# RupertLuo/Valley

Measured on AMD Instinct MI355X. Metric: frames/sec ViT-L/14 encode + prefill tokens/sec (13B), higher is better.
Workload: dtype bf16

## Files before the change

valley_amd/csrc/gemm_skinny.hip:

```cpp
#include <cstdlib>
#include "common.hpp"
#include "../../include/valley_hip.h"

namespace {

constexpr int SK_UNROLL = 4;

template <int EPI, int NWV>
__global__ void __launch_bounds__(NWV * 64) gemm_skinny_kernel(const uint16_t* __restrict__ A, const uint16_t* __restrict__ W,
                                                               const float* __restrict__ bias, uint16_t* __restrict__ C, int M, int N,
                                                               int K, int lda, int ldw, int ldc) {
    __shared__ f32x4 red[NWV][4][64];
    const int tid = threadIdx.x, lane = tid & 63, wave = tid >> 6;
    const int l15 = lane & 15, g = lane >> 4;
    const int n0 = blockIdx.x * 32, m0 = blockIdx.y * 32;
    const int kq = K / NWV, kbeg = wave * kq;
    const uint16_t* a0 = A + (size_t)min(m0 + l15, M - 1) * lda + kbeg + g * 8;
    const uint16_t* a1 = A + (size_t)min(m0 + 16 + l15, M - 1) * lda + kbeg + g * 8;
    const uint16_t* w0 = W + (size_t)(n0 + l15) * ldw + kbeg + g * 8;
    const uint16_t* w1 = W + (size_t)(n0 + 16 + l15) * ldw + kbeg + g * 8;
    f32x4 acc[2][2];
#pragma unroll
    for (int i = 0; i < 2; ++i)
#pragma unroll
// ... 56 lines not shown
                acc[0][0] = mfma16(fw0[u], fa0[u], acc[0][0]);
                acc[0][1] = mfma16(fw1[u], fa0[u], acc[0][1]);
                acc[1][0] = mfma16(fw0[u], fa1[u], acc[1][0]);
                acc[1][1] = mfma16(fw1[u], fa1[u], acc[1][1]);
            }
        }
    }
#pragma unroll
    for (int i = 0; i < 2; ++i)
#pragma unroll
        for (int j = 0; j < 2; ++j) red[wave][2 * i + j][lane] = acc[i][j];
    __syncthreads();
    if (wave >= 4) return;
    f32x4 v = red[0][wave][lane];
#pragma unroll
    for (int w = 1; w < NWV; ++w) v += red[w][wave][lane];
    const int m = m0 + (wave >> 1) * 16 + l15, n = n0 + (wave & 1) * 16 + 4 * g;
    if (m >= M) return;
    if (bias) v += *(const f32x4*)(bias + n);
    if constexpr (EPI == VLY_EPI_QUICK_GELU) {
#pragma unroll
        for (int r = 0; r < 4; ++r) v[r] = x_sigmoid(v[r], 1.702f);
    }
    if constexpr (EPI == VLY_EPI_RELU) {
#pragma unroll
        for (int r = 0; r < 4; ++r) v[r] = fmaxf(v[r], 0.f);
    }
    u32x2 pk;
    pk[0] = pack_h2(v[0], v[1]);
    pk[1] = pack_h2(v[2], v[3]);
    *(u32x2*)(C + (size_t)m * ldc + n) = pk;
}

}

extern "C" int vly_gemm_skinny_bf16(const void* A, const void* W, const float* bias, void* C, int M, int N, int K, int lda, int ldw,
                                    int ldc, int epilogue, void* stream) {
    if (M <= 0 || M > 256 || N <= 0 || N % 32 || K < 128 || K % 128 || (K >= 2048 && K % 512) || lda % 8 || ldw % 8 || ldc % 4 || ((uintptr_t)A & 15) ||
        ((uintptr_t)W & 15) || ((uintptr_t)C & 7) || (bias && ((uintptr_t)bias & 15))) {
        vly_set_error("vly_gemm_skinny_bf16: unsupported shape/alignment M=%d N=%d K=%d lda=%d ldw=%d ldc=%d", M, N, K, lda, ldw, ldc);
        return -22;
    }
    static const bool narrow_only = getenv("VLY_SKINNY_WAVES") && atoi(getenv("VLY_SKINNY_WAVES")) == 4;
    const bool wide = K >= 2048 && !narrow_only;
    dim3 grid(N / 32, (M + 31) / 32), block(wide ? 1024 : 256);
    hipStream_t st = (hipStream_t)stream;
#define VLY_SKINNY(E)                                                                                                      \
    do {                                                                                                                   \
        if (wide)                                                                                                          \
            hipLaunchKernelGGL((gemm_skinny_kernel<E, 16>), grid, block, 0, st, (const uint16_t*)A, (const uint16_t*)W, bias,  \
                               (uint16_t*)C, M, N, K, lda, ldw, ldc);                                                      \
        else                                                                                                               \
            hipLaunchKernelGGL((gemm_skinny_kernel<E, 4>), grid, block, 0, st, (const uint16_t*)A, (const uint16_t*)W, bias,   \
                               (uint16_t*)C, M, N, K, lda, ldw, ldc);                                                      \
    } while (0)
    switch (epilogue) {
        case VLY_EPI_NONE: VLY_SKINNY(VLY_EPI_NONE); break;
        case VLY_EPI_QUICK_GELU: VLY_SKINNY(VLY_EPI_QUICK_GELU); break;
        case VLY_EPI_RELU: VLY_SKINNY(VLY_EPI_RELU); break;
        default: vly_set_error("vly_gemm_skinny_bf16: unsupported epilogue %d", epilogue); return -22;
    }
#undef VLY_SKINNY
    return vly_check_launch("vly_gemm_skinny_bf16");
}
```

valley_amd/agpr_audit.py:

```python
import re
import subprocess

AUDITED = {"gemm_bf16.hip": "gemm_p4_kernel", "gemm_p32.hip": "gemm_p32_kernel", "gemm_p16.hip": "gemm_p16_kernel"}


def audit_asm(asm_path, kern):
    asm = open(asm_path).read().splitlines()
    bad = kernels = 0
    report = []
    i = 0
    areg = re.compile(r"\ba(\[(\d+|0x[0-9a-f]+)(:(\d+|0x[0-9a-f]+))?\]|\d+\b)")
    while i < len(asm):
        m = re.match(r"^(_ZN\S*" + kern + r"\S*):", asm[i])
        if not m:
            i += 1
            continue
        name = subprocess.run(["c++filt", m.group(1)], capture_output=True, text=True).stdout.strip()
        name = re.sub(r"\(anonymous namespace\)::", "", name).split("(")[0].replace("void ", "")
        j = i + 1
        in_asm = False
        outside, n_mfma, n_rd, n_mfma_compiler = [], 0, 0, 0
        while j < len(asm) and "s_endpgm" not in asm[j]:
            ln = asm[j]
            if ";;#ASMSTART" in ln:
                in_asm = True
            elif ";;#ASMEND" in ln:
                in_asm = False
            else:
                code = ln.split(";")[0]
                if in_asm:
                    if "v_mfma" in code:
                        n_mfma += 1
                    if "v_accvgpr_read" in code:
                        n_rd += 1
                elif areg.search(code) and not code.strip().startswith("."):
                    outside.append((j - i, code.strip()))
                    if "v_mfma" in code:
                        n_mfma_compiler += 1
                if "scratch_" in code:
                    outside.append((j - i, code.strip()))
            j += 1
        named = [int(x, 0) for ln in asm[i:j] for x in re.findall(r"\ba\[(?:\d+|0x[0-9a-f]+):(\d+|0x[0-9a-f]+)\]", ln.split(";")[0])]
        desc = "\n".join(asm[j:j + 120])
        nf = re.search(r"\.amdhsa_next_free_vgpr\s+(\d+)", desc)
        ao = re.search(r"\.amdhsa_accum_offset\s+(\d+)", desc)
        lit = n_mfma > 0 and n_mfma_compiler == 0 and "v_mfma" not in "\n".join(c for _, c in outside)
        if lit and named and nf and ao and int(nf.group(1)) - int(ao.group(1)) < max(named) + 1:
            outside.append((0, f"descriptor allocates {int(nf.group(1)) - int(ao.group(1))} accumulation registers, the asm names a{max(named)}"))
        if lit and not (nf and ao):
            outside.append((0, "kernel descriptor not found behind the kernel"))
        if n_mfma_compiler:
            lit = False
        if lit:
            kernels += 1
            status = "ok" if not outside else "FAIL"
            report.append(f"{name:48s} mfma {n_mfma:4d}  acc reads {n_rd:4d}  compiler AGPR / scratch instructions: {len(outside)}  {status}")
            for off, code in outside[:8]:
                report.append(f"    +{off}: {code}")
            bad += len(outside)
        i = j
    return report, kernels, bad
```

valley_amd/csrc/gemm_bf16.hip:

```cpp
#include <cmath>
#include <cstdlib>
#include <cstring>
#include <type_traits>
#include "common.hpp"
#include "../../include/valley_hip.h"

int vly_tile_order_m_fast(int M, int N, int K, int tiles_m, int tiles_n) {
    const double a = (double)M * K, w = (double)N * K;
    const double n_fast = a + w * (tiles_m < 8 ? tiles_m : 8);
    const double m_fast = w + a * (tiles_n < 8 ? tiles_n : 8);
    return m_fast < n_fast;
}

int vly_tile_group_height(int M, int N, int K, int tiles_m, int tiles_n, int BM, int BN, int wg_per_cu) {
    static const int forced = getenv("VLY_TILE_GM") ? atoi(getenv("VLY_TILE_GM")) : 0;
    static const int forced_max_m = getenv("VLY_TILE_GM_MAXM") ? atoi(getenv("VLY_TILE_GM_MAXM")) : 0x7fffffff;
    if (forced > 0 && M <= forced_max_m) return forced < tiles_m ? forced : tiles_m;
    static const bool grouped = !(getenv("VLY_TILE_GROUPED") && atoi(getenv("VLY_TILE_GROUPED")) == 0);
    if (!grouped) return vly_tile_order_m_fast(M, N, K, tiles_m, tiles_n) ? tiles_m : 1;
    if (tiles_n <= 8 && 8 % tiles_n == 0 && !vly_tile_order_m_fast(M, N, K, tiles_m, tiles_n)) return 1;
    const double conc = 32.0 * wg_per_cu;
    int gm = (int)(sqrt(conc * BN / BM) + 0.5);
    if (gm < 1) gm = 1;
    if (gm >= tiles_m || tiles_m <= gm + gm / 2) return tiles_m;
// ... 39 lines not shown
constexpr int P8_RD2_START = 1;
constexpr int P8_RD2_STRIDE = 2;
constexpr int P4_M0_LEAD = 2;
#ifndef VLY_P4_ROLL
#define VLY_P4_ROLL 1
#endif
#ifndef VLY_P4_ROLL_MASK
#define VLY_P4_ROLL_MASK 0x09
#endif
#ifndef VLY_P4_LIT
#define VLY_P4_LIT 1
#endif
#ifndef VLY_P4_CHAIN
#define VLY_P4_CHAIN 0
#endif
#ifndef VLY_P4_LATE
#define VLY_P4_LATE 0
#endif
#ifndef VLY_P4_DROPSTORE
#define VLY_P4_DROPSTORE 0
#endif
#ifndef VLY_P4_TIMING
#define VLY_P4_TIMING 0
#endif
#ifndef VLY_EXPERIMENTAL
#define VLY_EXPERIMENTAL 0
#endif

#if VLY_FP16
#define VLY_MFMA16_NAME "v_mfma_f32_16x16x32_f16"
#else
#define VLY_MFMA16_NAME "v_mfma_f32_16x16x32_bf16"
#endif
VLY_DEVICE void mfma16_lit(int blk, const bf16x8& a, const bf16x8& b) {
    asm volatile(VLY_MFMA16_NAME " a[%2:%3], %0, %1, a[%2:%3]" ::"v"(a), "v"(b), "i"(4 * blk), "i"(4 * blk + 3));
}
VLY_DEVICE void mfma16_lit_zero(int blk, const bf16x8& a, const bf16x8& b) {
    asm volatile(VLY_MFMA16_NAME " a[%2:%3], %0, %1, 0" ::"v"(a), "v"(b), "i"(4 * blk), "i"(4 * blk + 3));
}
VLY_DEVICE f32x4 acc_read_lit(int blk) {
    f32x4 v;
    asm volatile("v_accvgpr_read_b32 %0, a[%4]\n\tv_accvgpr_read_b32 %1, a[%5]\n\tv_accvgpr_read_b32 %2, a[%6]\n\tv_accvgpr_read_b32 %3, a[%7]"
                 : "=v"(v[0]), "=v"(v[1]), "=v"(v[2]), "=v"(v[3])
                 : "i"(4 * blk), "i"(4 * blk + 1), "i"(4 * blk + 2), "i"(4 * blk + 3));
    return v;
}
#define VLY_A8(n) "a" #n "0", "a" #n "1", "a" #n "2", "a" #n "3", "a" #n "4", "a" #n "5", "a" #n "6", "a" #n "7", "a" #n "8", "a" #n "9"
#define VLY_ALL_AGPRS                                                                                                                  \
    "a0", "a1", "a2", "a3", "a4", "a5", "a6", "a7", "a8", "a9", VLY_A8(1), VLY_A8(2), VLY_A8(3), VLY_A8(4), VLY_A8(5), VLY_A8(6), VLY_A8(7), \
        VLY_A8(8), VLY_A8(9), VLY_A8(10), VLY_A8(11), VLY_A8(12), VLY_A8(13), VLY_A8(14), VLY_A8(15), VLY_A8(16), VLY_A8(17), VLY_A8(18),   \
        VLY_A8(19), VLY_A8(20), VLY_A8(21), VLY_A8(22), VLY_A8(23), VLY_A8(24), "a250", "a251", "a252", "a253", "a254", "a255"

template <int MI, int NI, int N1, int S1, int D1, int N2, int S2, int D2, int N3, int S3, int D3, int N4, int S4, int D4, int MODE = 0,
          typename F1, typename F2, typename F3, typename F4, typename ACC>
VLY_DEVICE void phase_4w4(ACC& acc, const bf16x8 (&af)[MI], const bf16x8 (&wf)[NI], F1&& f1, F2&& f2, F3&& f3, F4&& f4) {
    __builtin_amdgcn_sched_barrier(0);
#pragma unroll
    for (int k = 0; k < N4; ++k)
        if (S4 + k * D4 < 0) f4(k);
#pragma unroll
    for (int i = 0; i < MI; ++i) {
#pragma unroll
        for (int j = 0; j < NI; ++j) {
            if constexpr (MODE == 3) mfma16_lit_zero(i * NI + j, wf[j], af[i]);
            else if constexpr (MODE == 2) mfma16_lit(i * NI + j, wf[j], af[i]);
            else acc[i][j] = mfma16(wf[j], af[i], acc[i][j]);
            const int t = i * NI + j;
            if (N1 > 0 && t >= S1 && (t - S1) % D1 == 0 && (t - S1) / D1 < N1) {
                __builtin_amdgcn_sched_barrier(0);
                f1((t - S1) / D1);
                __builtin_amdgcn_sched_barrier(0);
            }
            if (N3 > 0 && t >= S3 && (t - S3) % D3 == 0 && (t - S3) / D3 < N3) {
                __builtin_amdgcn_sched_barrier(0);
                f3((t - S3) / D3);
                __builtin_amdgcn_sched_barrier(0);
            }
            if (N4 > 0 && t >= S4 && (t - S4) % D4 == 0 && (t - S4) / D4 < N4) {
                __builtin_amdgcn_sched_barrier(0);
                f4((t - S4) / D4);
                __builtin_amdgcn_sched_barrier(0);
            }
            if (N2 > 0 && t >= S2 && (t - S2) % D2 == 0 && (t - S2) / D2 < N2) {
                __builtin_amdgcn_sched_barrier(0);
// ... 644 lines not shown
#undef VLY_FRAG_ROW
#undef VLY_FRAG_COL
#undef EPI_NH

VLY_DEVICE f32x4 acc_read(const f32x4& a) {
    f32x4 v;
    asm volatile("v_accvgpr_read_b32 %0, %4\n\tv_accvgpr_read_b32 %1, %5\n\tv_accvgpr_read_b32 %2, %6\n\tv_accvgpr_read_b32 %3, %7"
                 : "=v"(v[0]), "=v"(v[1]), "=v"(v[2]), "=v"(v[3])
                 : "a"(a[0]), "a"(a[1]), "a"(a[2]), "a"(a[3]));
    return v;
}
VLY_DEVICE void acc_read_pairs(const f32x4& a, f32x2& even, f32x2& odd) {
    asm volatile("v_accvgpr_read_b32 %0, %4\n\tv_accvgpr_read_b32 %1, %5\n\tv_accvgpr_read_b32 %2, %6\n\tv_accvgpr_read_b32 %3, %7"
                 : "=v"(even[0]), "=v"(odd[0]), "=v"(even[1]), "=v"(odd[1])
                 : "a"(a[0]), "a"(a[1]), "a"(a[2]), "a"(a[3]));
}

struct P4Cursor {
    int tile, k, kend, u, r;
};
constexpr int P4_SK_MAX_WAYS = 8;
constexpr unsigned P4_SK_SPIN_LIMIT = 1u << 24;
constexpr int P4_SK_ERR_FLAG = 4000;

template <int BM, int BN, int EPI, int OUT, bool SK>
__global__ void __launch_bounds__(256)
gemm_p4_kernel(const uint16_t* __restrict__ A, const uint16_t* __restrict__ W, const float* __restrict__ bias,
               const float* __restrict__ R, void* __restrict__ Cv, int M, int N, int K, int lda, int ldw, int ldc, int ldr,
               int tiles_m, int tiles_n, int gm, RopeArgs rp, float* __restrict__ slabs, unsigned* __restrict__ flags,
               unsigned epoch, int sk_S) {
    constexpr int WM = BM / 2, WN = BN / 2, NT = 256;
    constexpr bool SKT = SK && BM != 256;
    constexpr int MI = WM / 16, NI = WN / 16;
    constexpr int A_BYTES = BM * 128, W_BYTES = BN * 128, STAGE = A_BYTES + W_BYTES;
    constexpr int PA = BM * 8 / NT, PW = BN * 8 / NT, NS = PA + PW;
    static_assert(BM * 8 % NT == 0 && BN * 8 % NT == 0 && NI % 4 == 0, "tile/threads mismatch");
    constexpr int T = MI * NI, BAR_AT = MI + NI + P8_BAR_GAP, GL1_START = BAR_AT + 2;
    constexpr int GL_STRIDE = (2 * T - GL1_START) / NS;
    constexpr int N1 = (T - GL1_START + GL_STRIDE - 1) / GL_STRIDE, N2 = NS - N1;
    constexpr int GL2_START = GL1_START + N1 * GL_STRIDE - T;
    static_assert(GL1_START < T && GL_STRIDE >= 1 && N2 >= 0 && GL2_START + (N2 - 1) * GL_STRIDE < T, "piece schedule");
    __shared__ __attribute__((aligned(16))) char smem[2 * STAGE];
#if VLY_P4_TIMING
    __shared__ unsigned long long tstamp[64];
    int tsn = 0;
#define VLY_STAMP()                                                                            \
    do {                                                                                       \
        if (!SK && threadIdx.x == 0 && tsn < 64) tstamp[tsn] = __builtin_readcyclecounter();  \
        ++tsn;                                                                                 \
    } while (0)
#else
#define VLY_STAMP() do {} while (0)
#endif

    const int tid = threadIdx.x, lane = tid & 63;
    const int wave = __builtin_amdgcn_readfirstlane(tid >> 6);
    const int l15 = lane & 15, g = lane >> 4;
    const int ntiles = tiles_m * tiles_n, G = (int)gridDim.x;
    const int nk = K / BK;
    __builtin_assume(nk >= 2);
    const uint32_t wk = ldw < 0 ? (uint32_t)((N + 63) >> 6) * 4096u : (uint32_t)BK;
    auto tile_origin = [&](int t, int& m0, int& n0) {
        const int xcd = t & 7, qd = ntiles >> 3, rm = ntiles & 7;
        const int swz = (xcd < rm ? xcd * (qd + 1) : rm * (qd + 1) + (xcd - rm) * qd) + (t >> 3);
        const int gsz = gm * tiles_n, grp = swz / gsz, first = grp * gm;
        const int gh = min(gm, tiles_m - first), rr = swz - grp * gsz;
// ... 115 lines not shown
#pragma unroll
        for (int j = 0; j < NI; ++j) {
            w0[j] = *(const bf16x8*)(st + rdW + j * 2048 + sw0);
            w1[j] = *(const bf16x8*)(st + rdW + j * 2048 + sw1);
        }
#pragma unroll
        for (int i = 0; i < CH; ++i) {
            a0[i] = *(const bf16x8*)(st + rdA + i * 2048 + sw0);
            a1[i] = *(const bf16x8*)(st + rdA + i * 2048 + sw1);
        }
    };

#pragma unroll
    for (int q = 0; q < NS; ++q) piece(0, q);
    advance_load();
#pragma unroll
    for (int q = 0; q < NS; ++q) piece(1, q);
    advance_load();
    asm volatile("s_waitcnt vmcnt(%0)" ::"i"(NS) : "memory");
    __builtin_amdgcn_s_barrier();
    if constexpr (CHAIN) chain_preload(smem);
    else {
        auto r0 = rd_step0(smem);
#pragma unroll
        for (int k = 0; k < MI + NI; ++k) r0(k);
    }
    [[maybe_unused]] const __amdgpu_buffer_rsrc_t rsC =
        __builtin_amdgcn_make_buffer_rsrc(Cv, 0, (uint32_t)M * (uint32_t)ldc * (OUT == VLY_OUT_BF16 ? 2u : 4u), 0x00020000);
    int buf = 0;
    constexpr bool LIT = VLY_P4_LIT != 0 && !SK && OUT == VLY_OUT_BF16 && EPI != VLY_EPI_QKV_ROPE;
    constexpr bool ROLL = VLY_P4_ROLL != 0 && LIT && !CHAIN && ((VLY_P4_ROLL_MASK >> EPI) & 1) != 0;
    constexpr int NST_ = EPI == VLY_EPI_SWIGLU ? NI / 4 : NI / 2;
    static_assert(!ROLL || N1 + MI * NST_ <= 63, "vmcnt is a 6-bit count");
    if constexpr (LIT) asm volatile("" ::: VLY_ALL_AGPRS);
    f32x4 acc[MI][NI];
    bool wave_live = false;
    auto ktile = [&](auto first_c, bool relaxed = false) {
        constexpr bool FIRST = decltype(first_c)::value;
        const char* cur = smem + buf * STAGE;
        const char* nxt = smem + (buf ^ 1) * STAGE;
        __builtin_amdgcn_s_waitcnt(0xc07f);
        if constexpr (CHAIN) {
            if (wave_live) {
                phase_seq<CT1, CR1, 0, 1, CN1, CGL1, CGLS, 1, CBAR, 1, CN1, CGL1 - P4_M0_LEAD, CGLS>(
                    [&](int t) {
                        const int i = t / (2 * NI), j = (t % (2 * NI)) >> 1, st = t & 1;
                        if (FIRST && st == 0) mfma16_lit_zero(i * NI + j, w0[j], a0[i]);
                        else if (st == 0) mfma16_lit(i * NI + j, w0[j], a0[i]);
                        else mfma16_lit(i * NI + j, w1[j], a1[i]);
                    },
                    [&](int k) {
                        const int i = CH + (k >> 1);
                        if (k & 1) a1[i < MI ? i : 0] = *(const bf16x8*)(cur + rdA + i * 2048 + sw1);
                        else a0[i < MI ? i : 0] = *(const bf16x8*)(cur + rdA + i * 2048 + sw0);
                    },
                    [&](int q) { piece_ld(q); }, bar_a, [&](int q) { piece_m0(buf, q); });
            } else {
                __builtin_amdgcn_s_barrier();
#pragma unroll
                for (int q = 0; q < CN1; ++q) piece(buf, q);
            }
            asm volatile("s_waitcnt vmcnt(%0)" ::"i"(CN1) : "memory");
            __builtin_amdgcn_s_barrier();
            if (wave_live) {
                constexpr int CW = 2 * (MI - CH);
                phase_seq<CT2, 2 * CH, 1, 2, CN2, CGL2, CGLS, NI, CW - 1, CW, CN2, CGL2 - P4_M0_LEAD, CGLS>(
                    [&](int t) {
// ... 86 lines not shown
        if constexpr (OUT == VLY_OUT_BF16 && EPI != VLY_EPI_QKV_ROPE) {
            {
                const uint32_t rowb = (uint32_t)(em0 + wm0 + l15) * (uint32_t)ldc * 2u;
#pragma unroll
                for (int s = 0; s < NST; ++s) {
                    const int n = EPI == VLY_EPI_SWIGLU ? ((en0 + wn0) >> 1) + (4 * s + g) * 8
                                                        : en0 + wn0 + (2 * s + (g & 1)) * 16 + (g & 2) * 4;
                    vo[s] = rowb + (n + 8 <= No && !VLY_P4_DROPSTORE ? (uint32_t)n * 2u : 0x80000000u);
                }
            }
            if constexpr (EPI != VLY_EPI_SWIGLU) {
#pragma unroll
                for (int j = 0; j < NI; ++j) {
                    const int n = en0 + wn0 + j * 16 + g * 4;
                    bv[j] = f32x4{0.f, 0.f, 0.f, 0.f};
                    if (bias) bv[j] = *(const f32x4*)(bias + min(n, N - 4));
                }
            }
        }
    };
    [[maybe_unused]] auto epi_row = [&](int i, auto&& hook, auto defer_c) {
        constexpr bool DEFER = decltype(defer_c)::value;
        if constexpr (OUT == VLY_OUT_BF16 && EPI != VLY_EPI_QKV_ROPE) {
            if constexpr (EPI == VLY_EPI_SWIGLU) {
#pragma unroll
                for (int jq = 0; jq < NI / 4; ++jq) {
                    f32x2 gt[4], up[4], e[4];
#pragma unroll
                    for (int jj = 0; jj < 4; ++jj) {
                        if constexpr (SKT) {
                            const f32x4 v = acc_read(acc[i][4 * jq + jj]) + slab_term(i, 4 * jq + jj);
                            gt[jj] = f32x2{v[0], v[2]};
                            up[jj] = f32x2{v[1], v[3]};
                        } else if constexpr (LIT) {
                            const f32x4 v = acc_read_lit(i * NI + 4 * jq + jj);
                            gt[jj] = f32x2{v[0], v[2]};
                            up[jj] = f32x2{v[1], v[3]};
                        } else acc_read_pairs(acc[i][4 * jq + jj], gt[jj], up[jj]);
                    }
                    if constexpr (SKT) sk_next(i + 1, 4 * jq, 4);
                    hook(8 * jq + 0);
#pragma unroll
                    for (int q = 0; q < 4; ++q) e[q] = gt[q] * -1.4426950408889634f;
                    hook(8 * jq + 1);
#pragma unroll
                    for (int q = 0; q < 2; ++q) e[q] = f32x2{__builtin_amdgcn_exp2f(e[q][0]), __builtin_amdgcn_exp2f(e[q][1])};
                    hook(8 * jq + 2);
#pragma unroll
                    for (int q = 2; q < 4; ++q) e[q] = f32x2{__builtin_amdgcn_exp2f(e[q][0]), __builtin_amdgcn_exp2f(e[q][1])};
                    hook(8 * jq + 3);
#pragma unroll
                    for (int q = 0; q < 4; ++q) e[q] += 1.f;
#pragma unroll
                    for (int q = 0; q < 2; ++q) e[q] = f32x2{__builtin_amdgcn_rcpf(e[q][0]), __builtin_amdgcn_rcpf(e[q][1])};
                    hook(8 * jq + 4);
#pragma unroll
                    for (int q = 2; q < 4; ++q) e[q] = f32x2{__builtin_amdgcn_rcpf(e[q][0]), __builtin_amdgcn_rcpf(e[q][1])};
                    hook(8 * jq + 5);
#pragma unroll
                    for (int q = 0; q < 4; ++q) gt[q] *= e[q];
#pragma unroll
                    for (int q = 0; q < 4; ++q) gt[q] *= up[q];
                    hook(8 * jq + 6);
                    uint32_t d[4];
#pragma unroll
                    for (int jj = 0; jj < 4; ++jj) d[jj] = pack_h2(gt[jj][0], gt[jj][1]);
// ... 370 lines not shown
                    }
                }
            }
        }
        }
        if constexpr (SK) {
            if (!cur_next_seg(cc)) break;
            ct = cc.tile;
        } else {
            if (ct + G >= ntiles) break;
            ct += G;
        }
        tile_origin(ct, cm0, cn0);
        if constexpr (CHAIN) chain_preload(smem + buf * STAGE);
        else {
            auto r0 = rd_step0(smem + buf * STAGE);
#pragma unroll
            for (int k = 0; k < MI + NI; ++k) r0(k);
        }
    }
    VLY_STAMP();
    asm volatile("s_waitcnt vmcnt(0)" ::: "memory");
#if VLY_P4_TIMING
    VLY_STAMP();
    if (!SK && threadIdx.x == 0 && blockIdx.x < 64 && slabs) {
        unsigned long long* o = (unsigned long long*)slabs + (size_t)blockIdx.x * 65;
        o[0] = (unsigned long long)tsn;
        for (int q = 0; q < 64 && q < tsn; ++q) o[1 + q] = tstamp[q];
    }
#endif
}
#undef VLY_STAMP

#if VLY_P4_TIMING
static void* vlydbg_p4_buffer() {
    static void* buf = [] { void* p = nullptr; (void)hipMalloc(&p, 64 * 65 * 8); (void)hipMemset(p, 0, 64 * 65 * 8); return p; }();
    return buf;
}
extern "C" int vlydbg_p4_timing_read(unsigned long long* host) {
    return (int)hipMemcpy(host, vlydbg_p4_buffer(), 64 * 65 * 8, hipMemcpyDeviceToHost);
}
#endif
struct P4SkArgs {
    float* slabs;
    unsigned* flags;
    unsigned epoch;
    int slab_cap;
};

template <int BM, int BN, bool SK = false>
int launch_p4(const void* A, const void* W, const float* bias, const float* R, void* C, int M, int N, int K, int lda, int ldw,
              int ldc, int ldr, int epi, int out, hipStream_t st, const RopeArgs* rope = nullptr, const P4SkArgs* sk = nullptr) {
    const int tm = (M + BM - 1) / BM, tn = (N + BN - 1) / BN;
    const int gm = vly_tile_group_height(M, N, K, tm, tn, BM, BN, 1);
    const int No = epi == VLY_EPI_SWIGLU ? N >> 1 : N;
    const int vec_ok = (out == VLY_OUT_BF16 && ldc % 8 == 0 && ((uintptr_t)C & 15) == 0 && !R && No % 8 == 0 &&
                        (size_t)M * (size_t)ldc * 2 < ((size_t)1 << 31)) ? 1 : 0;
    if (out == VLY_OUT_BF16 && !vec_ok) return 1;
    static const int cus = [] {
        int dev = 0, n = 0;
        (void)hipGetDevice(&dev);
        (void)hipDeviceGetAttribute(&n, hipDeviceAttributeMultiprocessorCount, dev);
        if (getenv("VLY_P4_GRID")) n = atoi(getenv("VLY_P4_GRID"));
        return n > 0 ? n / 8 * 8 : 256;
    }();
    const int tiles = tm * tn;
    int sk_S = 1;
    if constexpr (SK) {
        const int rem = tiles % cus, rem8 = (rem + 7) & ~7, nk = K / BK;
        float best = 1e30f;
        for (int S = 1; S <= P4_SK_MAX_WAYS && rem > 0; ++S) {
            if (S > 1 && ((S - 1) * rem8 > sk->slab_cap || nk / S < 2 || (S - 1) * ((nk + S - 1) / S) >= nk)) continue;
            const float cost = (float)((S * rem8 + cus - 1) / cus) / (float)S + 0.06f * (float)(S - 1);
            if (cost < best - 1e-6f) { best = cost; sk_S = S; }
        }
        static const int pin = [] { const char* e = getenv("VLY_P4_SK_S"); return e ? atoi(e) : 0; }();
        if (pin > 0 && rem > 0 && (pin == 1 || ((pin - 1) * rem8 <= sk->slab_cap && nk / pin >= 2))) sk_S = pin;
    }
    dim3 grid(SK || tiles >= cus ? cus : tiles), block(256);
#if VLY_P4_TIMING
    P4SkArgs dbg{(float*)vlydbg_p4_buffer(), nullptr, 0u, 0};
    if (!sk) sk = &dbg;
#endif
#define VLY_P4_LAUNCH(E, O)                                                                                                  \
    hipLaunchKernelGGL((gemm_p4_kernel<BM, BN, E, O, SK>), grid, block, 0, st, (const uint16_t*)A, (const uint16_t*)W, bias, R, C, M, \
                       N, K, lda, ldw, ldc, ldr, tm, tn, gm, rope ? *rope : RopeArgs{}, sk ? sk->slabs : nullptr,                 \
                       sk ? sk->flags : nullptr, sk ? sk->epoch : 0u, sk_S)
    if (epi == VLY_EPI_NONE && out == VLY_OUT_BF16) VLY_P4_LAUNCH(VLY_EPI_NONE, VLY_OUT_BF16);
    else if (epi == VLY_EPI_NONE && out == VLY_OUT_F32) VLY_P4_LAUNCH(VLY_EPI_NONE, VLY_OUT_F32);
    else if (epi == VLY_EPI_QUICK_GELU && out == VLY_OUT_BF16) VLY_P4_LAUNCH(VLY_EPI_QUICK_GELU, VLY_OUT_BF16);
    else if (epi == VLY_EPI_SWIGLU && out == VLY_OUT_BF16) VLY_P4_LAUNCH(VLY_EPI_SWIGLU, VLY_OUT_BF16);
    else if (epi == VLY_EPI_RELU && out == VLY_OUT_BF16) VLY_P4_LAUNCH(VLY_EPI_RELU, VLY_OUT_BF16);
    else if (!SK && epi == VLY_EPI_QKV_ROPE && out == VLY_OUT_BF16 && rope) {
        if constexpr (!SK) VLY_P4_LAUNCH(VLY_EPI_QKV_ROPE, VLY_OUT_BF16);
    } else {
        vly_set_error("vly_gemm_bf16: unsupported epilogue/out_dtype combination (%d,%d) for the persistent tiles", epi, out);
        return -22;
    }
#undef VLY_P4_LAUNCH
    return vly_check_launch("vly_gemm_bf16");
}

template <int BM, int BN, int WM, int WN, int PIPE>
int launch_tile(const void* A, const void* W, const float* bias, const float* R, void* C, int M, int N, int K,
                int lda, int ldw, int ldc, int ldr, int epi, int out, hipStream_t st, void* C2 = nullptr,
                const RopeArgs* rope = nullptr) {
    constexpr int NT = (BM / WM) * (BN / WN) * 64;
    const int tm = (M + BM - 1) / BM, tn = (N + BN - 1) / BN;
    constexpr int STAGE_B = (BM + BN) * 128 * ((PIPE == 6 || PIPE == 7) ? 3 : 2);
    const int gm = vly_tile_group_height(M, N, K, tm, tn, BM, BN, STAGE_B <= 80 * 1024 ? 2 : 1);
    static const bool frag_only = getenv("VLY_EPILOGUE") && !strcmp(getenv("VLY_EPILOGUE"), "frag");
    static const bool lds_only = getenv("VLY_EPILOGUE") && !strcmp(getenv("VLY_EPILOGUE"), "lds");
    int wide = (out == VLY_OUT_BF16 && ldc % 8 == 0 && ((uintptr_t)C & 15) == 0 && !frag_only) ? 1 : 0;
    if (wide && PIPE == 8 && epi != VLY_EPI_QKV_ROPE && !lds_only) wide = 2;
    const int ksplit = C2 ? 2 : 1;
    dim3 grid(tm * tn * ksplit), block(NT);
#define VLY_GEMM_LAUNCH(E, O)                                                                         \
    hipLaunchKernelGGL((gemm_kernel<BM, BN, WM, WN, E, O, PIPE>), grid, block, 0, st, (const uint16_t*)A,   \
                       (const uint16_t*)W, bias, R, C, M, N, K, lda, ldw, ldc, ldr, tm, tn, gm, wide, ksplit, C2, rope ? *rope : RopeArgs{})
    if (epi == VLY_EPI_NONE && out == VLY_OUT_BF16) VLY_GEMM_LAUNCH(VLY_EPI_NONE, VLY_OUT_BF16);
    else if (epi == VLY_EPI_NONE && out == VLY_OUT_F32) VLY_GEMM_LAUNCH(VLY_EPI_NONE, VLY_OUT_F32);
    else if (epi == VLY_EPI_QUICK_GELU && out == VLY_OUT_BF16) VLY_GEMM_LAUNCH(VLY_EPI_QUICK_GELU, VLY_OUT_BF16);
    else if (epi == VLY_EPI_SWIGLU && out == VLY_OUT_BF16) VLY_GEMM_LAUNCH(VLY_EPI_SWIGLU, VLY_OUT_BF16);
    else if (epi == VLY_EPI_RELU && out == VLY_OUT_BF16) VLY_GEMM_LAUNCH(VLY_EPI_RELU, VLY_OUT_BF16);
    else if (epi == VLY_EPI_QKV_ROPE && out == VLY_OUT_BF16 && rope) {
        if constexpr (BN % 128 == 0) {
            if (!wide) { vly_set_error("vly_gemm_bf16_qkv_rope: qkv rows must be 16-byte aligned"); return -22; }
            VLY_GEMM_LAUNCH(VLY_EPI_QKV_ROPE, VLY_OUT_BF16);
        } else {
            vly_set_error("vly_gemm_bf16_qkv_rope: this tile is not a multiple of 128 columns wide");
            return -22;
        }
    }
// ... 97 lines not shown
        case 5: return launch_tile<192, 256, 96, 64, 0>(VLY_TILE_ARGS);
        case 73: return launch_tile<256, 128, 64, 64, 6>(VLY_TILE_ARGS);
        case 74: return launch_tile<128, 256, 64, 64, 6>(VLY_TILE_ARGS);
        case 76: return launch_tile<192, 192, 96, 48, 6>(VLY_TILE_ARGS);
        case 6: return launch_tile<192, 192, 96, 48, 0>(VLY_TILE_ARGS);
        case 83: return launch_tile<256, 128, 64, 64, 7>(VLY_TILE_ARGS);
        case 84: return launch_tile<128, 256, 64, 64, 7>(VLY_TILE_ARGS);
        case 86: return launch_tile<192, 192, 96, 48, 7>(VLY_TILE_ARGS);
        case 7: return launch_tile<128, 192, 64, 48, 0>(VLY_TILE_ARGS);
        case 8: return launch_tile<192, 128, 96, 32, 0>(VLY_TILE_ARGS);
        case 9: return launch_tile<256, 256, 64, 64, 0>(VLY_TILE_ARGS);
        case 93: return launch_tile<256, 128, 64, 32, 6>(VLY_TILE_ARGS);
        case 94: return launch_tile<128, 256, 32, 64, 6>(VLY_TILE_ARGS);
        case 497: {
            const int rc = rope || C2 ? 1 : valley_p16_gemm(A, W, bias, residual, C, M, N, K, lda, ldw, ldc, epilogue, out_dtype, st);
            return rc == 1 ? run_tile(197, tile_hint, VLY_TILE_ARGS_RAW) : rc;
        }
        case 397:
        case 398: {
            const int rc = rope || C2 ? 1 : valley_p32_gemm(A, W, bias, residual, C, M, N, K, lda, ldw, ldc, epilogue, out_dtype, st, t == 398);
            return rc == 1 ? run_tile(197, tile_hint, VLY_TILE_ARGS_RAW) : rc;
        }
        case 197:
        case 198:
        case 199:
            if (C2) { vly_set_error("vly_gemm_bf16: tile_hint %d does not take the split-K pair", tile_hint); return -22; }
            if (K < 2 * BK) return run_tile(t - 100, tile_hint, VLY_TILE_ARGS_RAW);
            {
                const int rc = t == 197 ? launch_p4<256, 256>(A, W, bias, residual, C, M, N, K, lda, ldw, ldc, ldr, epilogue, out_dtype, st, rope)
                               : t == 198 ? launch_p4<224, 256>(A, W, bias, residual, C, M, N, K, lda, ldw, ldc, ldr, epilogue, out_dtype, st, rope)
                                          : launch_p4<192, 256>(A, W, bias, residual, C, M, N, K, lda, ldw, ldc, ldr, epilogue, out_dtype, st, rope);
                return rc == 1 ? run_tile(t - 100, tile_hint, VLY_TILE_ARGS_RAW) : rc;
            }
        case 97:
        case 98:
        case 99:
            if (t == 97) return launch_tile<256, 256, 128, 128, 8>(VLY_TILE_ARGS);
            if (t == 98) return launch_tile<224, 256, 112, 128, 8>(VLY_TILE_ARGS);
            return launch_tile<192, 256, 96, 128, 8>(VLY_TILE_ARGS);
        case 51: return launch_tile<256, 256, 128, 64, 4>(VLY_TILE_ARGS);
        case 53: return launch_tile<256, 128, 64, 64, 4>(VLY_TILE_ARGS);
        case 54: return launch_tile<128, 256, 64, 64, 4>(VLY_TILE_ARGS);
        case 55: return launch_tile<192, 256, 96, 64, 4>(VLY_TILE_ARGS);
        default: vly_set_error("vly_gemm_bf16: bad tile_hint %d", tile_hint); return -22;
    }
#endif
#undef VLY_TILE_ARGS
#undef VLY_TILE_ARGS_RAW
}

extern "C" int vly_gemm_bf16(const void* A, const void* W, const float* bias, const float* residual, void* C,
                             int M, int N, int K, int lda, int ldw, int ldc, int ldr, int epilogue,
                             int out_dtype, int tile_hint, void* stream) {
    if (M <= 0 || N <= 0 || K <= 0) { vly_set_error("vly_gemm_bf16: empty problem"); return -22; }
    const bool wpacked = ldw == VLY_LDW_PACKED64;
    if (K % BK || lda % 8 || (ldw % 8 || (ldw <= 0 && !wpacked)) || N % 4 || ldc % 2 || (epilogue == VLY_EPI_SWIGLU && N % 8) ||
        ((uintptr_t)A & 15) || ((uintptr_t)W & 15) || ((uintptr_t)C & 7) ||
        (residual && (ldr % 4 || ((uintptr_t)residual & 15))) || (bias && ((uintptr_t)bias & 15))) {
        vly_set_error("vly_gemm_bf16: unsupported shape/alignment M=%d N=%d K=%d lda=%d ldw=%d ldc=%d ldr=%d",
                      M, N, K, lda, ldw, ldc, ldr);
        return -22;
    }
    if ((size_t)M * lda >= (1ull << 31) || (wpacked ? (size_t)((N + 63) / 64 * 64) * K : (size_t)N * ldw) >= (1ull << 31)) {
        vly_set_error("vly_gemm_bf16: operand exceeds 2^31 elements (32-bit byte offsets)");
        return -22;
    }
// ... 47 lines not shown
```

valley_amd/ops.py:

```python
from __future__ import annotations

import os
import threading
from typing import Optional

import torch

from . import lib as _lib
from . import runtime

EPI_NONE, EPI_QUICK_GELU, EPI_SWIGLU, EPI_RELU, EPI_QKV_ROPE = 0, 1, 2, 3, 4
OUT_BF16, OUT_F32 = 0, 1
POOL_MEAN, POOL_MAX, POOL_IMPORTANCE = 0, 1, 2


_RECORDER = None
TILE_NAMES = {1: "256, 256, 128, 64", 2: "128, 128, 64, 64", 3: "256, 128, 64, 64", 4: "128, 256, 64, 64",
              5: "192, 256, 96, 64", 6: "192, 192, 96, 48", 7: "128, 192, 64, 48",
              8: "192, 128, 96, 32", 9: "256, 256, 64, 64"}
TILE_SPECIAL = {93: ("256, 128, 64, 32", 6), 94: ("128, 256, 32, 64", 6),
                97: ("256, 256, 128, 128", 8), 98: ("224, 256, 112, 128", 8),
                99: ("192, 256, 96, 128", 8),
                197: ("p4 256, 256", 8), 198: ("p4 224, 256", 8), 199: ("p4 192, 256", 8)}

# ... 47 lines not shown

def _gemm_common(fn_name, a, w, bias, residual, epilogue, out_dtype, out, extra):
    _chk(a, runtime.HALF, "a", contiguous=False)
    wt, ldw = _w_args(w, fn_name == "vly_gemm_bf16" or (fn_name == "vly_gemm_bf16_streamk" and extra[0] in (297, 298, 299)))
    assert a.dim() == 2 and len(w.shape) == 2 and a.stride(1) == 1 and a.shape[1] == w.shape[1], (a.shape, w.shape)
    M, K = a.shape
    N = w.shape[0]
    No = N // 2 if epilogue == EPI_SWIGLU else N
    if out is None:
        out = torch.empty((M, No), dtype=out_dtype, device=a.device)
    else:
        assert tuple(out.shape) == (M, No) and out.stride(1) == 1, (out.shape, (M, No))
    if bias is not None:
        _chk(bias, torch.float32, "bias")
    if residual is not None:
        _chk(residual, torch.float32, "residual", contiguous=False)
        assert tuple(residual.shape) == (M, N) and residual.stride(1) == 1
    od = OUT_F32 if out.dtype == torch.float32 else OUT_BF16
    L = _lib.load()
    fn = getattr(L, fn_name)
    rec = _RECORDER if fn_name in ("vly_gemm_bf16", "vly_gemm_bf16_streamk") else None
    if rec is not None:
        sk = fn_name.endswith("streamk")
        tile = extra[0] or (L.vly_gemm_streamk_tile_for(M, N, K) if sk else L.vly_gemm_tile_for(M, N))
        if sk and tile not in (297, 298, 299):
            sk_loop = {0: "2, 0", 4: "2, 0", 5: "2, 1", 7: "3, 0", 8: "3, 1"}[tile % 100 // 10]
            tile %= 10
        e0, e1 = torch.cuda.Event(enable_timing=True), torch.cuda.Event(enable_timing=True)
        e0.record()
    rc = fn(a.data_ptr(), wt.data_ptr(), _ptr(bias), _ptr(residual), out.data_ptr(), M, N, K, a.stride(0), ldw,
            out.stride(0), residual.stride(0) if residual is not None else 0, epilogue, od, *extra, _stream())
    if rec is not None:
        e1.record()
        if sk and tile in (297, 298, 299):
            name = f"gemm_p4_kernel<{TILE_SPECIAL[tile - 100][0][3:]}, {epilogue}, {od}, true>"
        elif sk:
            name = f"gemm_sk_kernel<{TILE_NAMES[tile]}, {epilogue}, {od}, {sk_loop}>"
        elif tile in (197, 198, 199) and K >= 128 and (od == OUT_F32 or (residual is None and out.stride(0) % 8 == 0 and out.data_ptr() % 16 == 0)):
            name = f"gemm_p4_kernel<{TILE_SPECIAL[tile][0][3:]}, {epilogue}, {od}, false>"
        elif tile in TILE_SPECIAL:
            name = f"gemm_kernel<{TILE_SPECIAL[tile - 100 if tile in (197, 198, 199) else tile][0]}, {epilogue}, {od}, {TILE_SPECIAL[tile][1]}>"
        else:
            name = f"gemm_kernel<{TILE_NAMES[tile % 10]}, {epilogue}, {od}, {({0: 0, 1: 1, 3: 3, 5: 4, 7: 6, 8: 7})[tile // 10]}>"
        rec.append((name, 2.0 * M * N * K, e0, e1, (M, N, K, epilogue)))
    _lib.check(rc, fn_name)
    return out


def gemm_mfma(a, w, bias=None, residual=None, epilogue=EPI_NONE, out_dtype=None, out=None, tile_hint=0):
    out_dtype = runtime.HALF if out_dtype is None else out_dtype
    return _gemm_common("vly_gemm_bf16", a, w, bias, residual, epilogue, out_dtype, out, (tile_hint,))


_SK_WS = {}
_SK_OWNER = {}
_SK_POLL = {}
_SK_LOCK = threading.Lock()


def _sk_workspace(device):
    key = (device.index, int(torch.cuda.current_stream(device).cuda_stream))
    ent = _SK_WS.get(key)
    if ent is None:
        nbytes = _lib.load().vly_gemm_streamk_workspace_bytes()
        ent = [torch.zeros((nbytes + 15) // 16 * 4, dtype=torch.int32, device=device), 0]
        _SK_WS[key] = ent
    ent[1] = ent[1] % 0xFFFFFFF0 + 1
# ... 184 lines not shown
    for e in ents:
        M, N, K, epi, dt, hb, hr = e["key"][:7]
        _TUNED[(M, N, K, epi, _DT[dt], bool(hb), bool(hr)) + tuple(e["key"][7:])] = (e["kind"], e["tile"])
    return len(ents)


def save_tune_cache(path: str) -> None:
    import json
    ents = [{"key": [k[0], k[1], k[2], k[3], str(k[4]), k[5], k[6], *k[7:]], "kind": v[0], "tile": v[1]} for k, v in _TUNED.items()]
    tmp = f"{path}.{os.getpid()}.tmp"
    with open(tmp, "w") as f:
        json.dump(ents, f, indent=0)
    os.replace(tmp, path)


_TUNE_TABLE = os.path.join(os.path.dirname(os.path.abspath(__file__)), "tuned", "gfx950.json")
if os.environ.get("VALLEY_TUNE_TABLE", "1") != "0":
    load_tune_cache(_TUNE_TABLE)
if _TUNE_CACHE:
    load_tune_cache(_TUNE_CACHE)


_FLUSH = {}


def _flush_caches(device):
    buf = _FLUSH.get(device.index)
    if buf is None:
        buf = torch.empty(512 << 20, dtype=torch.uint8, device=device)
        _FLUSH[device.index] = buf
    buf.zero_()


CANDIDATES = [("tile", t) for t in (1, 2, 3, 4, 5, 6, 7, 8, 9, 51, 53, 54, 55, 73, 74, 76, 83, 84, 86, 93, 94, 97, 98, 99, 197, 198, 199)] + \
             [("sk", t) for t in (51, 55, 73, 74, 76, 83, 84, 86, 151, 155, 183, 184, 186, 298, 299)] + \
             ([("sk", 297)] if _lib.EXPERIMENTAL else [])
TUNE_TRIALS = int(os.environ.get("VALLEY_TUNE_TRIALS", "3"))
TUNE_FINALISTS = 4
_ONLINE = {}
_TUNE_LOCK = threading.RLock()
_STREAMS_SEEN = set()


TUNE_ONLINE = os.environ.get("VALLEY_TUNE_ONLINE", "1") != "0"


def _no_trials() -> bool:
    return _multi_stream() or not TUNE_ONLINE


def _multi_stream() -> bool:
    _STREAMS_SEEN.add(int(torch.cuda.current_stream().cuda_stream))
    return len(_STREAMS_SEEN) > 1


def _tune_key(M, N, K, epi, dtype, has_bias, has_res, w):
    k = (M, N, K, epi, torch.float32 if dtype == torch.float32 else "half", has_bias, has_res)
    return k + ("p64",) if isinstance(w, PackedWeight) else k


def tuning_pending() -> int:
    return len(_ONLINE)


def gemm_mfma_splitk2(a, w, bias, out, out2, tile_hint=0):
    _chk(a, runtime.HALF, "a", contiguous=False)
    wt, ldw = _w_args(w, True)
# ... 708 lines not shown
```

Before: 1704.

## Add templated skinny GEMM with shape-dependent tile and split-K wave configs

Adds a generalized gemm_rows_kernel, templated on the M/N tile, wave count and unroll depth, with double-buffered register loads and a shared-memory split-K reduction. The dispatcher routes most skinny shapes to it: a 16-row tile for small N, a 64x32 tile with 8 waves for wide N, and a 16-row tile with 8 waves for large K. The aim is to match tile size and K-split to each shape, so that small M wastes fewer MFMA rows and weight-load bandwidth is used better. Smaller tiles launch more blocks and reload A more often, and the 64-row variant raises register pressure.

```diff
diff --git a/valley_amd/csrc/gemm_skinny.hip b/valley_amd/csrc/gemm_skinny.hip
--- a/valley_amd/csrc/gemm_skinny.hip
+++ b/valley_amd/csrc/gemm_skinny.hip
@@ -112,6 +112,82 @@
     *(u32x2*)(C + (size_t)m * ldc + n) = pk;
 }
 
+template <int EPI, int MB, int NB, int NWV, int U>
+__global__ void __launch_bounds__(NWV * 64) gemm_rows_kernel(const uint16_t* __restrict__ A, const uint16_t* __restrict__ W,
+                                                             const float* __restrict__ bias, uint16_t* __restrict__ C, int M, int N,
+                                                             int K, int lda, int ldw, int ldc) {
+    constexpr int FM = MB / 16, FN = NB / 16, NF = FM * FN;
+    __shared__ f32x4 red[NWV][NF][64];
+    const int tid = threadIdx.x, lane = tid & 63, wave = tid >> 6;
+    const int l15 = lane & 15, g = lane >> 4;
+    const int n0 = blockIdx.x * NB, m0 = blockIdx.y * MB;
+    const int kq = K / NWV, kbeg = wave * kq;
+    const uint16_t* ap[FM];
+    const uint16_t* wp[FN];
+#pragma unroll
+    for (int i = 0; i < FM; ++i) ap[i] = A + (size_t)min(m0 + 16 * i + l15, M - 1) * lda + kbeg + g * 8;
+#pragma unroll
+    for (int j = 0; j < FN; ++j) wp[j] = W + (size_t)(n0 + 16 * j + l15) * ldw + kbeg + g * 8;
+    f32x4 acc[FM][FN];
+#pragma unroll
+    for (int i = 0; i < FM; ++i)
+#pragma unroll
+        for (int j = 0; j < FN; ++j) acc[i][j] = f32x4{0.f, 0.f, 0.f, 0.f};
+    bf16x8 fa[2][U][FM], fw[2][U][FN];
+    auto load_group = [&](int b, int k) {
+#pragma unroll
+        for (int u = 0; u < U; ++u) {
+#pragma unroll
+            for (int j = 0; j < FN; ++j) fw[b][u][j] = *(const bf16x8*)(wp[j] + k + 32 * u);
+#pragma unroll
+            for (int i = 0; i < FM; ++i) fa[b][u][i] = *(const bf16x8*)(ap[i] + k + 32 * u);
+        }
+    };
+    auto mfma_group = [&](int b) {
+#pragma unroll
+        for (int u = 0; u < U; ++u)
+#pragma unroll
+            for (int i = 0; i < FM; ++i)
+#pragma unroll
+                for (int j = 0; j < FN; ++j) acc[i][j] = mfma16(fw[b][u][j], fa[b][u][i], acc[i][j]);
+    };
+    const int groups = kq / (32 * U);
+    load_group(0, 0);
+#pragma unroll 1
+    for (int it = 0; it < groups; it += 2) {
+        if (it + 1 < groups) load_group(1, (it + 1) * 32 * U);
+        mfma_group(0);
+        if (it + 1 >= groups) break;
+        if (it + 2 < groups) load_group(0, (it + 2) * 32 * U);
+        mfma_group(1);
+    }
+#pragma unroll
+    for (int i = 0; i < FM; ++i)
+#pragma unroll
+        for (int j = 0; j < FN; ++j) red[wave][FN * i + j][lane] = acc[i][j];
+    __syncthreads();
+    for (int f = wave; f < NF; f += NWV) {
+        f32x4 v = red[0][f][lane];
+#pragma unroll
+        for (int w = 1; w < NWV; ++w) v += red[w][f][lane];
+        const int m = m0 + (f / FN) * 16 + l15, n = n0 + (f % FN) * 16 + 4 * g;
+        if (m >= M) continue;
+        if (bias) v += *(const f32x4*)(bias + n);
+        if constexpr (EPI == VLY_EPI_QUICK_GELU) {
+#pragma unroll
+            for (int r = 0; r < 4; ++r) v[r] = x_sigmoid(v[r], 1.702f);
+        }
+        if constexpr (EPI == VLY_EPI_RELU) {
+#pragma unroll
+            for (int r = 0; r < 4; ++r) v[r] = fmaxf(v[r], 0.f);
+        }
+        u32x2 pk;
+        pk[0] = pack_h2(v[0], v[1]);
+        pk[1] = pack_h2(v[2], v[3]);
+        *(u32x2*)(C + (size_t)m * ldc + n) = pk;
+    }
+}
+
 }
 
 extern "C" int vly_gemm_skinny_bf16(const void* A, const void* W, const float* bias, void* C, int M, int N, int K, int lda, int ldw,
@@ -123,11 +199,21 @@
     }
     static const bool narrow_only = getenv("VLY_SKINNY_WAVES") && atoi(getenv("VLY_SKINNY_WAVES")) == 4;
     const bool wide = K >= 2048 && !narrow_only;
+    const int rows = K >= 2048 ? (K % 1024 == 0 ? 3 : 0) : K % 512 == 0 ? (N >= 4096 ? 2 : 1) : 0;
+    hipStream_t st = (hipStream_t)stream;
+#define VLY_ROWS(E, MB, NB, NWV, U)                                                                                        \
+    hipLaunchKernelGGL((gemm_rows_kernel<E, MB, NB, NWV, U>), dim3(N / NB, (M + MB - 1) / MB), dim3(NWV * 64), 0, st,     \
+                       (const uint16_t*)A, (const uint16_t*)W, bias, (uint16_t*)C, M, N, K, lda, ldw, ldc)
     dim3 grid(N / 32, (M + 31) / 32), block(wide ? 1024 : 256);
-    hipStream_t st = (hipStream_t)stream;
 #define VLY_SKINNY(E)                                                                                                      \
     do {                                                                                                                   \
-        if (wide)                                                                                                          \
+        if (rows == 1)                                                                                                     \
+            VLY_ROWS(E, 16, 32, 4, 4);                                                                                     \
+        else if (rows == 2)                                                                                                \
+            VLY_ROWS(E, 64, 32, 8, 2);                                                                                     \
+        else if (rows == 3)                                                                                                \
+            VLY_ROWS(E, 16, 32, 8, 4);                                                                                     \
+        else if (wide)                                                                                                     \
             hipLaunchKernelGGL((gemm_skinny_kernel<E, 16>), grid, block, 0, st, (const uint16_t*)A, (const uint16_t*)W, bias,  \
                                (uint16_t*)C, M, N, K, lda, ldw, ldc);                                                      \
         else                                                                                                               \
@@ -141,5 +227,6 @@
         default: vly_set_error("vly_gemm_skinny_bf16: unsupported epilogue %d", epilogue); return -22;
     }
 #undef VLY_SKINNY
+#undef VLY_ROWS
     return vly_check_launch("vly_gemm_skinny_bf16");
 }
```

Result: no change. 1705 (median of 6 runs) (+0.1%).

## Add 192x384 SwiGLU p4 GEMM tile with overflow accumulators in named VGPRs

Applied to the files above, without the earlier changes.

Adds a larger 192x384 tile variant of the p4 GEMM kernel for the SwiGLU epilogue. Its 72 accumulator blocks exceed the 256 AGPRs, so blocks beyond 64 are held in named arch VGPRs v224-v255, which are declared clobbered. The aim is more operand reuse per loaded tile in the gate/up projection. The variant is exposed as tile 194 to the autotuner, and the AGPR audit script is extended to check the VGPR accumulator blocks. The cost is heavier register pressure on the compiler-allocated VGPRs, with a risk of spills or lower occupancy.

```diff
diff --git a/valley_amd/agpr_audit.py b/valley_amd/agpr_audit.py
--- a/valley_amd/agpr_audit.py
+++ b/valley_amd/agpr_audit.py
@@ -51,12 +51,61 @@
             outside.append((0, "kernel descriptor not found behind the kernel"))
         if n_mfma_compiler:
             lit = False
+        vbad, n_vacc = _audit_vgpr_blocks(asm[i + 1:j], desc) if lit else ([], 0)
+        outside += vbad
         if lit:
             kernels += 1
             status = "ok" if not outside else "FAIL"
-            report.append(f"{name:48s} mfma {n_mfma:4d}  acc reads {n_rd:4d}  compiler AGPR / scratch instructions: {len(outside)}  {status}")
+            report.append(f"{name:48s} mfma {n_mfma:4d}  acc reads {n_rd:4d}  compiler AGPR / scratch instructions: {len(outside)}  {status}"
+                          + (f"  (+{n_vacc} accumulation VGPRs by name)" if n_vacc else ""))
             for off, code in outside[:8]:
                 report.append(f"    +{off}: {code}")
             bad += len(outside)
         i = j
     return report, kernels, bad
+
+
+_VREG = re.compile(r"\bv(?:\[(\d+|0x[0-9a-f]+)(?::(\d+|0x[0-9a-f]+))?\]|(\d+)\b)")
+
+
+def _vregs(code):
+    return [(int(a, 0), int(b or a, 0)) if a else (int(c), int(c)) for a, b, c in _VREG.findall(code)]
+
+
+def _audit_vgpr_blocks(body, desc):
+    lines, in_asm = [], False
+    for k, ln in enumerate(body):
+        if ";;#ASMSTART" in ln:
+            in_asm = True
+        elif ";;#ASMEND" in ln:
+            in_asm = False
+        else:
+            code = ln.split(";")[0].strip()
+            if code and not code.startswith("."):
+                lines.append((k + 1, code, in_asm))
+    dsts = [_vregs(c)[0] for _, c, a in lines if a and c.startswith("v_mfma") and re.match(r"v_mfma\S*\s+v\[", c)]
+    if not dsts:
+        return [], 0
+    base = min(d[0] for d in dsts)
+    top = max(d[1] for d in dsts)
+    bad = []
+    for off, code, in_asm in lines:
+        regs = [r for r in _vregs(code) if r[1] >= base]
+        if not regs:
+            continue
+        if not in_asm:
+            bad.append((off, code))
+        elif code.startswith("v_mfma"):
+            ops = _vregs(code)
+            if len(ops) < 3 or ops[1][1] >= base or ops[2][1] >= base or (len(ops) > 3 and ops[3] != ops[0]):
+                bad.append((off, code))
+        elif code.startswith("v_mov_b32"):
+            ops = _vregs(code)
+            if len(ops) != 2 or ops[0][1] >= base or ops[1][0] < base:
+                bad.append((off, code))
+        else:
+            bad.append((off, code))
+    ao = re.search(r"\.amdhsa_accum_offset\s+(\d+)", desc)
+    if not ao or int(ao.group(1)) < top + 1:
+        bad.append((0, f"descriptor's arch VGPRs ({ao.group(1) if ao else '?'}) do not cover v{top} the asm accumulates into"))
+    return bad, top + 1 - base
diff --git a/valley_amd/csrc/gemm_bf16.hip b/valley_amd/csrc/gemm_bf16.hip
--- a/valley_amd/csrc/gemm_bf16.hip
+++ b/valley_amd/csrc/gemm_bf16.hip
@@ -95,11 +95,14 @@
 #else
 #define VLY_MFMA16_NAME "v_mfma_f32_16x16x32_bf16"
 #endif
+constexpr int VLY_VACC0 = 224;
 VLY_DEVICE void mfma16_lit(int blk, const bf16x8& a, const bf16x8& b) {
-    asm volatile(VLY_MFMA16_NAME " a[%2:%3], %0, %1, a[%2:%3]" ::"v"(a), "v"(b), "i"(4 * blk), "i"(4 * blk + 3));
+    if (blk < 64) asm volatile(VLY_MFMA16_NAME " a[%2:%3], %0, %1, a[%2:%3]" ::"v"(a), "v"(b), "i"(4 * blk), "i"(4 * blk + 3));
+    else asm volatile(VLY_MFMA16_NAME " v[%2:%3], %0, %1, v[%2:%3]" ::"v"(a), "v"(b), "i"(VLY_VACC0 + 4 * (blk - 64)), "i"(VLY_VACC0 + 4 * (blk - 64) + 3));
 }
 VLY_DEVICE void mfma16_lit_zero(int blk, const bf16x8& a, const bf16x8& b) {
-    asm volatile(VLY_MFMA16_NAME " a[%2:%3], %0, %1, 0" ::"v"(a), "v"(b), "i"(4 * blk), "i"(4 * blk + 3));
+    if (blk < 64) asm volatile(VLY_MFMA16_NAME " a[%2:%3], %0, %1, 0" ::"v"(a), "v"(b), "i"(4 * blk), "i"(4 * blk + 3));
+    else asm volatile(VLY_MFMA16_NAME " v[%2:%3], %0, %1, 0" ::"v"(a), "v"(b), "i"(VLY_VACC0 + 4 * (blk - 64)), "i"(VLY_VACC0 + 4 * (blk - 64) + 3));
 }
 VLY_DEVICE f32x4 acc_read_lit(int blk) {
     f32x4 v;
@@ -108,11 +111,22 @@
                  : "i"(4 * blk), "i"(4 * blk + 1), "i"(4 * blk + 2), "i"(4 * blk + 3));
     return v;
 }
+VLY_DEVICE f32x4 acc_read_vlit(int blk) {
+    f32x4 v;
+    asm volatile("v_mov_b32 %0, v[%4]\n\tv_mov_b32 %1, v[%5]\n\tv_mov_b32 %2, v[%6]\n\tv_mov_b32 %3, v[%7]"
+                 : "=v"(v[0]), "=v"(v[1]), "=v"(v[2]), "=v"(v[3])
+                 : "i"(VLY_VACC0 + 4 * (blk - 64)), "i"(VLY_VACC0 + 4 * (blk - 64) + 1), "i"(VLY_VACC0 + 4 * (blk - 64) + 2),
+                   "i"(VLY_VACC0 + 4 * (blk - 64) + 3));
+    return v;
+}
 #define VLY_A8(n) "a" #n "0", "a" #n "1", "a" #n "2", "a" #n "3", "a" #n "4", "a" #n "5", "a" #n "6", "a" #n "7", "a" #n "8", "a" #n "9"
 #define VLY_ALL_AGPRS                                                                                                                  \
     "a0", "a1", "a2", "a3", "a4", "a5", "a6", "a7", "a8", "a9", VLY_A8(1), VLY_A8(2), VLY_A8(3), VLY_A8(4), VLY_A8(5), VLY_A8(6), VLY_A8(7), \
         VLY_A8(8), VLY_A8(9), VLY_A8(10), VLY_A8(11), VLY_A8(12), VLY_A8(13), VLY_A8(14), VLY_A8(15), VLY_A8(16), VLY_A8(17), VLY_A8(18),   \
         VLY_A8(19), VLY_A8(20), VLY_A8(21), VLY_A8(22), VLY_A8(23), VLY_A8(24), "a250", "a251", "a252", "a253", "a254", "a255"
+#define VLY_V8(n) "v" #n "0", "v" #n "1", "v" #n "2", "v" #n "3", "v" #n "4", "v" #n "5", "v" #n "6", "v" #n "7", "v" #n "8", "v" #n "9"
+#define VLY_VACC_VGPRS                                                                                                                 \
+    "v224", "v225", "v226", "v227", "v228", "v229", VLY_V8(23), VLY_V8(24), "v250", "v251", "v252", "v253", "v254", "v255"
 
 template <int MI, int NI, int N1, int S1, int D1, int N2, int S2, int D2, int N3, int S3, int D3, int N4, int S4, int D4, int MODE = 0,
           typename F1, typename F2, typename F3, typename F4, typename ACC>
@@ -823,6 +837,7 @@
     constexpr int WM = BM / 2, WN = BN / 2, NT = 256;
     constexpr bool SKT = SK && BM != 256;
     constexpr int MI = WM / 16, NI = WN / 16;
+    constexpr bool VACC = MI * NI > 64;
     constexpr int A_BYTES = BM * 128, W_BYTES = BN * 128, STAGE = A_BYTES + W_BYTES;
     constexpr int PA = BM * 8 / NT, PW = BN * 8 / NT, NS = PA + PW;
     static_assert(BM * 8 % NT == 0 && BN * 8 % NT == 0 && NI % 4 == 0, "tile/threads mismatch");
@@ -1004,7 +1019,10 @@
     constexpr bool ROLL = VLY_P4_ROLL != 0 && LIT && !CHAIN && ((VLY_P4_ROLL_MASK >> EPI) & 1) != 0;
     constexpr int NST_ = EPI == VLY_EPI_SWIGLU ? NI / 4 : NI / 2;
     static_assert(!ROLL || N1 + MI * NST_ <= 63, "vmcnt is a 6-bit count");
+    static_assert(!VACC || (LIT && !ROLL && !CHAIN && EPI == VLY_EPI_SWIGLU && MI * NI <= 64 + (256 - VLY_VACC0) / 4),
+                  "VGPR accumulator blocks: by name, unrolled schedule, SwiGLU epilogue");
     if constexpr (LIT) asm volatile("" ::: VLY_ALL_AGPRS);
+    if constexpr (VACC) asm volatile("" ::: VLY_VACC_VGPRS);
     f32x4 acc[MI][NI];
     bool wave_live = false;
     auto ktile = [&](auto first_c, bool relaxed = false) {
@@ -1157,6 +1175,11 @@
                             const f32x4 v = acc_read(acc[i][4 * jq + jj]) + slab_term(i, 4 * jq + jj);
                             gt[jj] = f32x2{v[0], v[2]};
                             up[jj] = f32x2{v[1], v[3]};
+                        } else if constexpr (VACC) {
+                            const int blk = i * NI + 4 * jq + jj;
+                            const f32x4 v = blk < 64 ? acc_read_lit(blk) : acc_read_vlit(blk);
+                            gt[jj] = f32x2{v[0], v[2]};
+                            up[jj] = f32x2{v[1], v[3]};
                         } else if constexpr (LIT) {
                             const f32x4 v = acc_read_lit(i * NI + 4 * jq + jj);
                             gt[jj] = f32x2{v[0], v[2]};
@@ -1593,6 +1616,12 @@
 }
 #undef VLY_STAMP
 
+#ifdef VLY_FEW_TILES
+#define VLY_P4V 0
+#else
+#define VLY_P4V (VLY_P4_LIT != 0 && VLY_P4_CHAIN == 0 && !(VLY_P4_ROLL != 0 && ((VLY_P4_ROLL_MASK >> VLY_EPI_SWIGLU) & 1)))
+#endif
+
 #if VLY_P4_TIMING
 static void* vlydbg_p4_buffer() {
     static void* buf = [] { void* p = nullptr; (void)hipMalloc(&p, 64 * 65 * 8); (void)hipMemset(p, 0, 64 * 65 * 8); return p; }();
@@ -1608,6 +1637,17 @@
     unsigned epoch;
     int slab_cap;
 };
+
+int p4_cus() {
+    static const int cus = [] {
+        int dev = 0, n = 0;
+        (void)hipGetDevice(&dev);
+        (void)hipDeviceGetAttribute(&n, hipDeviceAttributeMultiprocessorCount, dev);
+        if (getenv("VLY_P4_GRID")) n = atoi(getenv("VLY_P4_GRID"));
+        return n > 0 ? n / 8 * 8 : 256;
+    }();
+    return cus;
+}
 
 template <int BM, int BN, bool SK = false>
 int launch_p4(const void* A, const void* W, const float* bias, const float* R, void* C, int M, int N, int K, int lda, int ldw,
@@ -1618,13 +1658,7 @@
     const int vec_ok = (out == VLY_OUT_BF16 && ldc % 8 == 0 && ((uintptr_t)C & 15) == 0 && !R && No % 8 == 0 &&
                         (size_t)M * (size_t)ldc * 2 < ((size_t)1 << 31)) ? 1 : 0;
     if (out == VLY_OUT_BF16 && !vec_ok) return 1;
-    static const int cus = [] {
-        int dev = 0, n = 0;
-        (void)hipGetDevice(&dev);
-        (void)hipDeviceGetAttribute(&n, hipDeviceAttributeMultiprocessorCount, dev);
-        if (getenv("VLY_P4_GRID")) n = atoi(getenv("VLY_P4_GRID"));
-        return n > 0 ? n / 8 * 8 : 256;
-    }();
+    const int cus = p4_cus();
     const int tiles = tm * tn;
     int sk_S = 1;
     if constexpr (SK) {
@@ -1660,6 +1694,24 @@
     }
 #undef VLY_P4_LAUNCH
     return vly_check_launch("vly_gemm_bf16");
+}
+
+int launch_p4v(const void* A, const void* W, const float* bias, const float* R, void* C, int M, int N, int K, int lda, int ldw, int ldc,
+               int ldr, int epi, int out, hipStream_t st) {
+#if VLY_P4V
+    constexpr int BM = 192, BN = 384;
+    if (epi != VLY_EPI_SWIGLU || out != VLY_OUT_BF16 || bias || R || ldc % 8 || ((uintptr_t)C & 15) || (N >> 1) % 8 ||
+        (size_t)M * (size_t)ldc * 2 >= ((size_t)1 << 31))
+        return 1;
+    const int tm = (M + BM - 1) / BM, tn = (N + BN - 1) / BN, tiles = tm * tn, cus = p4_cus();
+    const int gm = vly_tile_group_height(M, N, K, tm, tn, BM, BN, 1);
+    hipLaunchKernelGGL((gemm_p4_kernel<BM, BN, VLY_EPI_SWIGLU, VLY_OUT_BF16, false>), dim3(tiles >= cus ? cus : tiles), dim3(256), 0, st, (const uint16_t*)A, (const uint16_t*)W, bias, R, C,
+                       M, N, K, lda, ldw, ldc, ldr, tm, tn, gm, RopeArgs{}, nullptr, nullptr, 0u, 1);
+    return vly_check_launch("vly_gemm_bf16");
+#else
+    (void)A, (void)W, (void)bias, (void)R, (void)C, (void)M, (void)N, (void)K, (void)lda, (void)ldw, (void)ldc, (void)ldr, (void)epi, (void)out, (void)st;
+    return 1;
+#endif
 }
 
 template <int BM, int BN, int WM, int WN, int PIPE>
@@ -1823,6 +1875,12 @@
                                           : launch_p4<192, 256>(A, W, bias, residual, C, M, N, K, lda, ldw, ldc, ldr, epilogue, out_dtype, st, rope);
                 return rc == 1 ? run_tile(t - 100, tile_hint, VLY_TILE_ARGS_RAW) : rc;
             }
+        case 194:
+            if (C2) { vly_set_error("vly_gemm_bf16: tile_hint %d does not take the split-K pair", tile_hint); return -22; }
+            {
+                const int rc = K < 2 * BK || rope ? 1 : launch_p4v(A, W, bias, residual, C, M, N, K, lda, ldw, ldc, ldr, epilogue, out_dtype, st);
+                return rc == 1 ? run_tile(197, tile_hint, VLY_TILE_ARGS_RAW) : rc;
+            }
         case 97:
         case 98:
         case 99:
diff --git a/valley_amd/ops.py b/valley_amd/ops.py
--- a/valley_amd/ops.py
+++ b/valley_amd/ops.py
@@ -103,7 +103,13 @@
             out.stride(0), residual.stride(0) if residual is not None else 0, epilogue, od, *extra, _stream())
     if rec is not None:
         e1.record()
-        if sk and tile in (297, 298, 299):
+        p4v = (not sk and tile == 194 and epilogue == EPI_SWIGLU and od == OUT_BF16 and bias is None and residual is None and K >= 128
+               and out.stride(0) % 8 == 0 and out.data_ptr() % 16 == 0)
+        if not sk and tile == 194 and not p4v:
+            tile = 197
+        if p4v:
+            name = f"gemm_p4_kernel<192, 384, {epilogue}, {od}, false>"
+        elif sk and tile in (297, 298, 299):
             name = f"gemm_p4_kernel<{TILE_SPECIAL[tile - 100][0][3:]}, {epilogue}, {od}, true>"
         elif sk:
             name = f"gemm_sk_kernel<{TILE_NAMES[tile]}, {epilogue}, {od}, {sk_loop}>"
@@ -354,7 +360,7 @@
     buf.zero_()
 
 
-CANDIDATES = [("tile", t) for t in (1, 2, 3, 4, 5, 6, 7, 8, 9, 51, 53, 54, 55, 73, 74, 76, 83, 84, 86, 93, 94, 97, 98, 99, 197, 198, 199)] + \
+CANDIDATES = [("tile", t) for t in (1, 2, 3, 4, 5, 6, 7, 8, 9, 51, 53, 54, 55, 73, 74, 76, 83, 84, 86, 93, 94, 97, 98, 99, 194, 197, 198, 199)] + \
              [("sk", t) for t in (51, 55, 73, 74, 76, 83, 84, 86, 151, 155, 183, 184, 186, 298, 299)] + \
              ([("sk", 297)] if _lib.EXPERIMENTAL else [])
 TUNE_TRIALS = int(os.environ.get("VALLEY_TUNE_TRIALS", "3"))
```

New measurement: 1727 before, 1758 after, median of 6. +1.8%, better.
